# facebook/winterfell

Hardware: NVIDIA H100
Metric: prover_ms (lower is better)
Workload: dtype u64

## Files before the change

include/winterfell_b200.h:

```cpp
#ifndef WINTERFELL_B200_H
#define WINTERFELL_B200_H

#include <stddef.h>
#include <stdint.h>

#ifdef __cplusplus
extern "C" {
#endif

#define WF_OK 0
#define WF_ERR_CUDA (-1)
#define WF_ERR_INVALID (-2)
#define WF_ERR_UNSUPPORTED (-3)
#define WF_ERR_STATE (-4)

#define WF_HASH_BLAKE3_256 0
#define WF_HASH_RP64_256 1
#define WF_HASH_RPJIVE64_256 2
#define WF_HASH_SHA3_256 4
#define WF_HASH_BLAKE3_192 3

typedef struct wf_ctx wf_ctx;
typedef struct wf_mat wf_mat;
typedef struct wf_tree wf_tree;
// ... 62 lines not shown
typedef int (*wf_aux_builder_fn)(void* user, const uint64_t* rand_elements, uint64_t* aux_out);
int wf_prove_air_aux(wf_ctx* ctx, const uint64_t* air_desc, size_t air_desc_len, const uint64_t* const* trace_cols, int mont,
                     uint32_t log_n, const uint32_t* opts, wf_aux_builder_fn aux_builder, void* aux_user, uint8_t* proof,
                     size_t* proof_len);

typedef int (*wf_aux_assertions_fn)(void* user, const uint64_t* rand_elements, uint64_t* values);
int wf_prove_air_aux_dyn(wf_ctx* ctx, const uint64_t* air_desc, size_t air_desc_len, const uint64_t* const* trace_cols, int mont,
                         uint32_t log_n, const uint32_t* opts, wf_aux_builder_fn aux_builder, wf_aux_assertions_fn aux_assertions,
                         void* aux_user, uint8_t* proof, size_t* proof_len);

int wf_prove_fib_dev(wf_ctx* ctx, const uint64_t* d_trace, uint32_t k, uint32_t log_n, const uint64_t* results,
                     const uint32_t* opts, uint8_t* proof, size_t* proof_len);

int wf_aux_build_check(const uint64_t* air_desc, size_t air_desc_len, const uint64_t* aux_build, size_t aux_build_len, uint32_t log_n,
                       char* msg, size_t msg_cap);
int wf_aux_build(wf_ctx* ctx, const uint64_t* air_desc, size_t air_desc_len, const uint64_t* aux_build, size_t aux_build_len,
                 const wf_mat* main_evals, const uint64_t* rand, uint32_t ext, wf_mat** aux);
int wf_prove_air_aux_built(wf_ctx* ctx, const uint64_t* air_desc, size_t air_desc_len, const uint64_t* aux_build, size_t aux_build_len,
                           const uint64_t* const* trace_cols, const uint64_t* d_trace, int mont, uint32_t log_n, const uint32_t* opts,
                           wf_aux_assertions_fn aux_assertions, void* aux_user, uint8_t* proof, size_t* proof_len);

int wf_eval_constraints(wf_ctx* ctx, const uint64_t* air_desc, size_t air_desc_len, uint32_t log_n, uint32_t blowup, uint32_t ext,
                        const wf_mat* main_lde, const wf_mat* aux_lde, const uint64_t* coeffs, const uint64_t* aux_rand,
                        wf_mat** out);
int wf_composition_commit(wf_ctx* ctx, int hash_id, const wf_mat* comp_trace, uint32_t log_n, uint32_t blowup, uint32_t ext,
                          uint32_t num_cols, wf_mat** polys, wf_mat** lde, wf_tree** tree);
int wf_composition_commit_partitioned(wf_ctx* ctx, int hash_id, const wf_mat* comp_trace, uint32_t log_n, uint32_t blowup,
                                      uint32_t ext, uint32_t num_cols, uint32_t partition_size, wf_mat** polys, wf_mat** lde,
                                      wf_tree** tree);
int wf_mat_evaluate_at(wf_ctx* ctx, const wf_mat* polys, uint32_t ext, uint32_t col_ext, const uint64_t* z0, const uint64_t* z1,
                       uint64_t* out0, uint64_t* out1);
int wf_deep_compose(wf_ctx* ctx, uint32_t ext, const wf_mat* main_lde, const wf_mat* aux_lde, const wf_mat* cons_lde, uint32_t log_n,
                    const uint64_t* z, const uint64_t* coeffs, const uint64_t* ood_cur, const uint64_t* ood_next, wf_mat** out);

int wf_grind(wf_ctx* ctx, int hash_id, const uint8_t seed[32], uint32_t grinding, uint64_t* nonce);

typedef struct wf_comm {
    void* user;
    int rank, world;
    int (*exchange)(void* user, size_t nsend, const int* send_peer, const void* const* send, size_t nrecv,
                    const int* recv_peer, void* const* recv, size_t bytes);
    int (*all_gather_host)(void* user, const void* send, void* recv, size_t bytes);
    int (*all_reduce_sum)(void* user, void* d_buf, size_t words);
    int (*fork)(void* user);
    int (*join)(void* user);
} wf_comm;
int wf_prove_fib_sharded(wf_ctx* ctx, const wf_comm* comm, const uint64_t* const* local_cols, const uint64_t* d_local, int mont,
                         uint32_t k, uint32_t log_n, const uint64_t* results, const uint32_t* opts, uint8_t* proof,
                         size_t* proof_len, double* stats);

int wf_ctx_set_jit(wf_ctx* ctx, int on);
int wf_ctx_jit_stats(wf_ctx* ctx, uint64_t* compiled, uint64_t* cache_hits, uint64_t* fallbacks);
int wf_jit_compile_air(const uint64_t* air_desc, size_t air_desc_len, uint32_t ext, size_t* cubin_bytes, char* log, size_t log_cap);
int wf_air_check(const uint64_t* air_desc, size_t air_desc_len, uint32_t log_n, uint32_t blowup, char* msg, size_t msg_cap);

int wf_ntt_dev(wf_ctx* ctx, uint64_t* d_data, uint32_t log_n, uint32_t cols, int inverse);
int wf_hash_rows_dev(wf_ctx* ctx, int hash_id, const uint64_t* d_rows, size_t nrows, uint32_t cols, uint8_t* d_digests);
int wf_merkle_dev(wf_ctx* ctx, int hash_id, const uint8_t* d_leaves, size_t nleaves, uint8_t* d_nodes);
int wf_fri_fold_dev(wf_ctx* ctx, const uint64_t* d_evals, size_t len, int ext_degree, uint32_t folding_factor,
                    const uint64_t* alpha, uint64_t* d_next);

#define WF_FIELD_TEST_SHIFTS {1, 3, 6, 12, 24, 31, 32, 33, 48, 63, 64, 65, 72, 80, 84, 90, 95, 96}
int wf_field_ops_dev(wf_ctx* ctx, const uint64_t* d_a, const uint64_t* d_b, size_t n, uint64_t* d_out);
int wf_ext_ops_dev(wf_ctx* ctx, uint32_t ext, const uint64_t* d_a, const uint64_t* d_b, size_t n, uint64_t* d_out);

int wf_host_hash_elements(int hash_id, const uint64_t* elems, size_t n, uint8_t out[32]);
// ... 19 lines not shown
```

winterfell_b200/__init__.py:

```python
import ctypes as C
import os

import numpy as np

_HERE = os.path.dirname(os.path.abspath(__file__))
LIB_PATH = os.environ.get("WF_LIB_PATH") or os.path.join(_HERE, "libwinterfell_b200.so")

P = 0xFFFFFFFF00000001
HASH_BLAKE3_256 = 0
HASH_RP64_256 = 1
HASH_RPJIVE64_256 = 2
HASH_BLAKE3_192 = 3
HASH_SHA3_256 = 4

WF_OK = 0

u64p = C.POINTER(C.c_uint64)
u8p = C.POINTER(C.c_uint8)
vp = C.c_void_p

FRI_COMMIT_FN = C.CFUNCTYPE(None, C.c_void_p, u8p)
FRI_DRAW_FN = C.CFUNCTYPE(None, C.c_void_p, u64p)
AUX_BUILDER = C.CFUNCTYPE(C.c_int, C.c_void_p, u64p, u64p)

# ... 25 lines not shown
    ("wf_mat_wrap_device", C.c_int, [vp, vp, C.c_size_t, C.c_uint32, C.POINTER(vp)]),
    ("wf_trace_lde_from_host", C.c_int, [vp, C.POINTER(u64p), C.c_uint32, C.c_size_t, C.c_int, C.c_uint32, C.POINTER(vp), C.POINTER(vp)]),
    ("wf_mat_interpolate_with_offset", C.c_int, [vp, vp, C.c_uint64, C.POINTER(vp)]),
    ("wf_commit_rows", C.c_int, [vp, C.c_int, vp, C.POINTER(vp)]),
    ("wf_commit_rows_partitioned", C.c_int, [vp, C.c_int, vp, C.c_uint32, C.POINTER(vp)]),
    ("wf_tree_from_leaves", C.c_int, [vp, C.c_int, vp, C.c_size_t, C.c_int, C.POINTER(vp)]),
    ("wf_tree_free", C.c_int, [vp, vp]),
    ("wf_tree_root", C.c_int, [vp, vp, u8p]),
    ("wf_tree_num_leaves", C.c_size_t, [vp]),
    ("wf_tree_to_host", C.c_int, [vp, vp, u8p, u8p]),
    ("wf_tree_open_many", C.c_int, [vp, vp, u64p, C.c_size_t, u8p, u8p, C.POINTER(C.c_size_t)]),
    ("wf_fri_build_layers", C.c_int, [vp, C.c_int, vp, C.c_int, C.c_uint32, C.c_uint32, C.c_uint32, FRI_COMMIT_FN, FRI_DRAW_FN, vp, C.POINTER(vp)]),
    ("wf_fri_build_layers_default_channel", C.c_int, [vp, C.c_int, vp, C.c_int, C.c_uint32, C.c_uint32, C.c_uint32, u8p, C.c_size_t, C.POINTER(vp)]),
    ("wf_fri_num_layers", C.c_uint32, [vp]),
    ("wf_fri_remainder", C.c_size_t, [vp, u64p, C.c_size_t]),
    ("wf_fri_build_proof", C.c_int, [vp, vp, u64p, C.c_size_t, u8p, C.POINTER(C.c_size_t)]),
    ("wf_fri_free", C.c_int, [vp, vp]),
    ("wf_prove_fib", C.c_int, [vp, C.POINTER(u64p), C.c_int, C.c_uint32, C.c_uint32, u64p, C.POINTER(C.c_uint32), u8p, C.POINTER(C.c_size_t)]),
    ("wf_prove_air", C.c_int, [vp, u64p, C.c_size_t, C.POINTER(u64p), C.c_int, C.c_uint32, C.POINTER(C.c_uint32), u8p, C.POINTER(C.c_size_t)]),
    ("wf_prove_air_aux", C.c_int, [vp, u64p, C.c_size_t, C.POINTER(u64p), C.c_int, C.c_uint32, C.POINTER(C.c_uint32), AUX_BUILDER, vp,
                                   u8p, C.POINTER(C.c_size_t)]),
        ("wf_prove_air_aux_dyn", C.c_int, [vp, u64p, C.c_size_t, C.POINTER(u64p), C.c_int, C.c_uint32, C.POINTER(C.c_uint32), AUX_BUILDER, AUX_BUILDER, vp,
                                   u8p, C.POINTER(C.c_size_t)]),
    ("wf_aux_build_check", C.c_int, [u64p, C.c_size_t, u64p, C.c_size_t, C.c_uint32, C.c_char_p, C.c_size_t]),
    ("wf_aux_build", C.c_int, [vp, u64p, C.c_size_t, u64p, C.c_size_t, vp, u64p, C.c_uint32, C.POINTER(vp)]),
    ("wf_prove_air_aux_built", C.c_int, [vp, u64p, C.c_size_t, u64p, C.c_size_t, C.POINTER(u64p), vp, C.c_int, C.c_uint32,
                                         C.POINTER(C.c_uint32), AUX_BUILDER, vp, u8p, C.POINTER(C.c_size_t)]),
    ("wf_eval_constraints", C.c_int, [vp, u64p, C.c_size_t, C.c_uint32, C.c_uint32, C.c_uint32, vp, vp, u64p, u64p, C.POINTER(vp)]),
    ("wf_composition_commit", C.c_int, [vp, C.c_int, vp, C.c_uint32, C.c_uint32, C.c_uint32, C.c_uint32, C.POINTER(vp), C.POINTER(vp), C.POINTER(vp)]),
    ("wf_composition_commit_partitioned", C.c_int, [vp, C.c_int, vp, C.c_uint32, C.c_uint32, C.c_uint32, C.c_uint32, C.c_uint32, C.POINTER(vp),
                                                    C.POINTER(vp), C.POINTER(vp)]),
    ("wf_mat_evaluate_at", C.c_int, [vp, vp, C.c_uint32, C.c_uint32, u64p, u64p, u64p, u64p]),
    ("wf_deep_compose", C.c_int, [vp, C.c_uint32, vp, vp, vp, C.c_uint32, u64p, u64p, u64p, u64p, C.POINTER(vp)]),
    ("wf_prove_fib_dev", C.c_int, [vp, vp, C.c_uint32, C.c_uint32, u64p, C.POINTER(C.c_uint32), u8p, C.POINTER(C.c_size_t)]),
    ("wf_grind", C.c_int, [vp, C.c_int, u8p, C.c_uint32, C.POINTER(C.c_uint64)]),
    ("wf_ntt_dev", C.c_int, [vp, vp, C.c_uint32, C.c_uint32, C.c_int]),
    ("wf_hash_rows_dev", C.c_int, [vp, C.c_int, vp, C.c_size_t, C.c_uint32, vp]),
    ("wf_merkle_dev", C.c_int, [vp, C.c_int, vp, C.c_size_t, vp]),
    ("wf_fri_fold_dev", C.c_int, [vp, vp, C.c_size_t, C.c_int, C.c_uint32, u64p, vp]),
    ("wf_field_ops_dev", C.c_int, [vp, vp, vp, C.c_size_t, vp]),
    ("wf_ext_ops_dev", C.c_int, [vp, C.c_uint32, vp, vp, C.c_size_t, vp]),
    ("wf_ctx_set_jit", C.c_int, [vp, C.c_int]),
    ("wf_ctx_jit_stats", C.c_int, [vp, C.POINTER(C.c_uint64), C.POINTER(C.c_uint64), C.POINTER(C.c_uint64)]),
    ("wf_jit_compile_air", C.c_int, [u64p, C.c_size_t, C.c_uint32, C.POINTER(C.c_size_t), C.c_char_p, C.c_size_t]),
    ("wf_air_check", C.c_int, [u64p, C.c_size_t, C.c_uint32, C.c_uint32, C.c_char_p, C.c_size_t]),
    ("wf_host_hash_elements", C.c_int, [C.c_int, u64p, C.c_size_t, u8p]),
    ("wf_host_merge", C.c_int, [C.c_int, u8p, u8p]),
    ("wf_host_merge_with_int", C.c_int, [C.c_int, u8p, C.c_uint64, u8p]),
    ("wf_host_mul", C.c_uint64, [C.c_uint64, C.c_uint64]),
    ("wf_host_mul_2exp", C.c_uint64, [C.c_uint64, C.c_uint32]),
    ("wf_host_mont_to_canonical", C.c_uint64, [C.c_uint64]),
    ("wf_host_canonical_to_mont", C.c_uint64, [C.c_uint64]),
    ("wf_host_write_usize", C.c_size_t, [C.c_uint64, u8p]),
    ("wf_host_coin_draw", C.c_int, [C.c_int, u64p, C.c_size_t, u8p, C.c_int, C.c_size_t, u64p]),
    ("wf_host_build_fib_trace", C.c_int, [C.c_uint32, C.c_size_t, u64p, u64p]),
    ("wf_host_sharded_opening_plan", C.c_long, [C.c_size_t, C.c_int, C.c_int, u64p, C.c_size_t, u64p, u64p, C.c_size_t]),
    ("wf_prove_fib_sharded", C.c_int, [vp, vp, C.POINTER(u64p), vp, C.c_int, C.c_uint32, C.c_uint32, u64p, C.POINTER(C.c_uint32), u8p,
                                       C.POINTER(C.c_size_t), C.POINTER(C.c_double)]),
]


def declared_symbols():
    return [s[0] for s in _SIGS]


def lib():
# ... 117 lines not shown
        d_, dp = _u64(desc)
        c_, cp = _u64(coeffs)
        rp = None
        if aux_rand is not None:
            r_, rp = _u64(aux_rand)
        h = vp()
        self.check(self.L.wf_eval_constraints(self.h, dp, d_.size, log_n, blowup, ext, main_lde.h, aux_lde.h if aux_lde else None,
                                              cp, rp, C.byref(h)))
        return Mat(self, h)

    def composition_commit(self, hash_id, comp_trace, log_n, blowup, ext, num_cols):
        a, b, t = vp(), vp(), vp()
        self.check(self.L.wf_composition_commit(self.h, hash_id, comp_trace.h, log_n, blowup, ext, num_cols,
                                                C.byref(a), C.byref(b), C.byref(t)))
        return Mat(self, a), Mat(self, b), Tree(self, t)

    def evaluate_at(self, polys, ext, col_ext, z0, z1):
        a_, ap = _u64(z0)
        b_, bp = _u64(z1)
        ncols = polys.cols // col_ext
        o0 = np.zeros((ncols, ext), dtype=np.uint64)
        o1 = np.zeros((ncols, ext), dtype=np.uint64)
        self.check(self.L.wf_mat_evaluate_at(self.h, polys.h, ext, col_ext, ap, bp, o0.ctypes.data_as(u64p), o1.ctypes.data_as(u64p)))
        return o0, o1

    def deep_compose(self, ext, main_lde, aux_lde, cons_lde, log_n, z, coeffs, ood_cur, ood_next):
        z_, zp = _u64(z)
        c_, cp = _u64(coeffs)
        a_, ap = _u64(ood_cur)
        b_, bp = _u64(ood_next)
        h = vp()
        self.check(self.L.wf_deep_compose(self.h, ext, main_lde.h, aux_lde.h if aux_lde else None, cons_lde.h, log_n, zp, cp, ap, bp,
                                          C.byref(h)))
        return Mat(self, h)

    def prove_fib(self, trace, results, opts, mont=False, out_buf=None):
        a = np.ascontiguousarray(trace, dtype=np.uint64)
        c, n = a.shape
        ptrs = (u64p * c)(*[a[j].ctypes.data_as(u64p) for j in range(c)])
        r_, rp = _u64(results)
        o_ = np.ascontiguousarray(opts, dtype=np.uint32)
        buf = out_buf if out_buf is not None else np.zeros(1 << 23, dtype=np.uint8)
        cap = buf.size
        ln = C.c_size_t(cap)
        self.check(self.L.wf_prove_fib(self.h, ptrs, int(mont), c // 2, int(n).bit_length() - 1, rp,
                                       o_.ctypes.data_as(C.POINTER(C.c_uint32)), buf.ctypes.data_as(u8p), C.byref(ln)))
        return buf[: ln.value].tobytes()

    def prove_air(self, desc, trace, opts, mont=False):
        d_, dp = _u64(desc)
        a = np.ascontiguousarray(trace, dtype=np.uint64)
        c, n = a.shape
        ptrs = (u64p * c)(*[a[j].ctypes.data_as(u64p) for j in range(c)])
        o_ = np.ascontiguousarray(opts, dtype=np.uint32)
        cap = 1 << 23
        buf = np.zeros(cap, dtype=np.uint8)
        ln = C.c_size_t(cap)
        self.check(self.L.wf_prove_air(self.h, dp, d_.size, ptrs, int(mont), int(n).bit_length() - 1,
                                       o_.ctypes.data_as(C.POINTER(C.c_uint32)), buf.ctypes.data_as(u8p), C.byref(ln)))
        return buf[: ln.value].tobytes()

    def prove_air_aux(self, desc, trace, opts, builder, aux_width, num_rands, mont=False):
        d_, dp = _u64(desc)
        a = np.ascontiguousarray(trace, dtype=np.uint64)
        c, n = a.shape
        ptrs = (u64p * c)(*[a[j].ctypes.data_as(u64p) for j in range(c)])
# ... 343 lines not shown
```

winterfell_b200/csrc/prover.cu:

```cuda
#include <algorithm>
#include <chrono>

#include "internal.hpp"
#include "blake3.cuh"
#include "alg_hash.cuh"

#include "constraints_generic.cuh"

#ifndef FIB_ROWS_D3
#define FIB_ROWS_D3 2
#endif
struct FibEvalParams {
    SegMatrix lde;
    SegMatrix out;
    u32 k, log_n, log_blowup, log_ce_blowup;
    const u64* coef;
    u64 K0[3], K1[3];
    const u64* tw_ce;
    u64 zt[8];
    u64 last;
    size_t row0, ce_rows;
};

template <int D>
// ... 232 lines not shown
            for (int q = 0; q < 8; q++) {
                u32 j = g * 8 + q;
                if (j < p.c) {
#pragma unroll
                    for (int d = 0; d < D; d++) acc_mad(acc[d], s_t[(size_t)j * D + d], v[q]);
                }
            }
        }
    } else {
        for (u32 j = 0; j < p.c; j++) {
            const u64 v = seg_at(p.trace, row, j);
#pragma unroll
            for (int d = 0; d < D; d++) acc_mad(acc[d], s_t[(size_t)j * D + d], v);
        }
    }
    GlExt<D> S;
#pragma unroll
    for (int d = 0; d < D; d++) S.v[d] = acc_reduce(acc[d]);
    for (u32 j = 0; j < p.aw; j++) {
        GlExt<D> av;
#pragma unroll
        for (int q = 0; q < D; q++) av.v[q] = seg_at(p.aux, row, j * D + q);
        S = ext_add(S, ext_mul(ld_ext<D>(s_a + (size_t)j * D), av));
    }
    for (u32 j = 0; j < p.kc; j++) {
        GlExt<D> hv;
#pragma unroll
        for (int q = 0; q < D; q++) hv.v[q] = seg_at(p.cons, row, j * D + q);
        S = ext_add(S, ext_mul(ld_ext<D>(s_c + (size_t)j * D), hv));
    }
    u64* o = p.out.base + row * p.out.W;
#pragma unroll
    for (int q = 0; q < D; q++) o[q] = S.v[q];
}

#ifndef DEEP_ROWS1
#define DEEP_ROWS1 8
#endif
#ifndef DEEP_ROWS2
#define DEEP_ROWS2 8
#endif
#ifndef DEEP_ROWS3
#define DEEP_ROWS3 8
#endif
#ifndef DEEP_DIV_MINB
#define DEEP_DIV_MINB 2
#endif
#define DEEP_ROWS (D == 1 ? DEEP_ROWS1 : (D == 2 ? DEEP_ROWS2 : DEEP_ROWS3))
template <int D>
struct DeepPoint {
    u64 t, s, n;
    GlExt<D> q1, q0;
};
template <int D>
__device__ __forceinline__ u64 deep_m(const DeepPoint<D>& pt, u64 x, u64 x2) {
    if (D == 1) return gl_sub(x, pt.n);
    if (D == 2) return gl_add(gl_sub(x2, gl_mul(pt.t, x)), pt.n);
    return gl_sub(gl_add(gl_mul(x2, gl_sub(x, pt.t)), gl_mul(pt.s, x)), pt.n);
}
template <int D>
__device__ __forceinline__ GlExt<D> deep_q(const DeepPoint<D>& pt, u64 x, u64 x2) {
    GlExt<D> q;
    if (D == 1) { q.v[0] = 1; return q; }
    if (D == 2) { q = ext_sub(ext_from_base<D>(x), pt.q0); return q; }
    q = ext_sub(pt.q0, ext_mul_base(pt.q1, x));
    q.v[0] = gl_add(q.v[0], x2);
// ... 31 lines not shown
    for (int r = 0; r < ROWS; r++) {
        size_t row = tid + r * stride;
        if (row >= N) continue;
        u64* o = p.out.base + row * p.out.W;
        const GlExt<D> S = ld_ext<D>(o);
        const u64 x = D > 1 ? xs[r] : 0, x2 = D > 1 ? gl_sqr(x) : 0;
        const GlExt<D> a = ext_mul_base(ext_mul(ext_sub(S, Sz), deep_q<D>(pz, x, x2)), den[2 * r]);
        const GlExt<D> b = ext_mul_base(ext_mul(ext_sub(S, Szg), deep_q<D>(pzg, x, x2)), den[2 * r + 1]);
        const GlExt<D> v = ext_add(a, b);
#pragma unroll
        for (int q = 0; q < D; q++) o[q] = v.v[q];
    }
}
template <int D>
static bool deep_point(const GlExt<D>& z, DeepPoint<D>& pt) {
    pt.t = pt.s = pt.n = 0;
    pt.q1 = ext_zero<D>(); pt.q0 = ext_zero<D>();
    if (D == 1) { pt.n = z.v[0]; return true; }
    const GlExt<D> z1 = ext_frobenius(z);
    if (D == 2) {
        const GlExt<D> tr = ext_add(z, z1), nm = ext_mul(z, z1);
        pt.t = tr.v[0]; pt.n = nm.v[0]; pt.q0 = z1;
        return tr.v[1] == 0 && nm.v[1] == 0;
    }
    const GlExt<D> z2 = ext_frobenius(z1);
    const GlExt<D> tr = ext_add(z, ext_add(z1, z2));
    const GlExt<D> z12 = ext_mul(z1, z2);
    const GlExt<D> sm = ext_add(ext_mul(z, ext_add(z1, z2)), z12), nm = ext_mul(z, z12);
    pt.t = tr.v[0]; pt.s = sm.v[0]; pt.n = nm.v[0];
    pt.q1 = ext_add(z1, z2); pt.q0 = z12;
    bool ok = true;
    for (int k = 1; k < D; k++) ok = ok && tr.v[k] == 0 && sm.v[k] == 0 && nm.v[k] == 0;
    return ok;
}

__global__ void __launch_bounds__(256) grind_kernel(int hash_id, const u64* seed , u64 start, u64 count, u32 grinding,
                                                    unsigned long long* result) {
    u64 idx = (u64)blockIdx.x * blockDim.x + threadIdx.x;
    if (idx >= count) return;
    u64 nonce = start + idx;
    u64 head;
    if (WF_HASH_IS_BLAKE3(hash_id)) {
        u32 ws[8], cv[8];
#pragma unroll
        for (int i = 0; i < 4; i++) { ws[2 * i] = (u32)seed[i]; ws[2 * i + 1] = (u32)(seed[i] >> 32); }
        if (hash_id == WF_HASH_BLAKE3_256) b3_merge_with_int_words<8>(ws, nonce, cv, b3_runtime_one());
        else b3_merge_with_int_words<6>(ws, nonce, cv, b3_runtime_one());
        head = (u64)cv[0] | ((u64)cv[1] << 32);
    } else {
        u64 sd[4], o[4];
#pragma unroll
        for (int i = 0; i < 4; i++) sd[i] = seed[i];
        if (hash_id == WF_HASH_RP64_256) alg_merge_with_int<WF_HASH_RP64_256>(sd, nonce, o);
        else if (hash_id == WF_HASH_SHA3_256) alg_merge_with_int<WF_HASH_SHA3_256>(sd, nonce, o);
        else alg_merge_with_int<WF_HASH_RPJIVE64_256>(sd, nonce, o);
        head = o[0];
    }
    u64 mask = grinding >= 64 ? ~0ULL : ((1ULL << grinding) - 1);
    if ((head & mask) == 0) atomicMin(result, (unsigned long long)nonce);
}

static int grind_on_device(wf_ctx* ctx, int hash_id, const Digest& seed, u32 grinding, u64* nonce_out) {
    if (grinding == 0) { *nonce_out = 1; return WF_OK; }
    void *d_seed, *d_res;
    CKI(wf_dev_alloc(ctx, 32, &d_seed));
    CKI(wf_dev_alloc(ctx, 8, &d_res));
// ... 554 lines not shown
    CK(cudaGetLastError());
    wf_mat_free(ctx, ccoefs);
    wf_mark(ctx, "composition_interpolate");
    *polys_out = cpolys;
    return WF_OK;
}
int composition_commit(wf_ctx* ctx, int h, const wf_mat* comp, u32 log_n, u32 log_b, int D, u32 kc, wf_mat** polys_out,
                       wf_mat** lde_out, wf_tree** tree_out, u32 partition_words = 0) {
    wf_mat *cpolys = nullptr, *clde = nullptr;
    CKI(composition_polys(ctx, comp, log_n, D, kc, &cpolys));
    int r = wf_mat_lde(ctx, cpolys, log_b, &clde);
    if (r == WF_OK) {
        wf_mark(ctx, "composition_lde");
        if (tree_out) r = wf_commit_rows_partitioned(ctx, h, clde, partition_words, tree_out);
    }
    if (r != WF_OK) { wf_mat_free(ctx, cpolys); wf_mat_free(ctx, clde); return r; }
    *polys_out = cpolys;
    *lde_out = clde;
    return WF_OK;
}

template <int D>
int deep_compose(wf_ctx* ctx, const wf_mat* lde, const wf_mat* alde, const wf_mat* clde, u32 kc, u32 log_N,
                 const std::vector<GlExt<D>>& dc, const GlExt<D>& z, const GlExt<D>& zg, const GlExt<D>& Sz, const GlExt<D>& Szg,
                 wf_mat** out, size_t row0 = 0, size_t nrows = 0) {
    const u32 c = lde->m.cols, aw = alde ? alde->m.cols / D : 0, ct = c + aw;
    const size_t N = nrows ? nrows : ((size_t)1 << log_N);
    u64 *d_dt, *d_dq, *d_da;
    CKI(upload_ext<D>(ctx, dc, 0, ct + kc, &d_dt));
    d_da = d_dt + (size_t)c * D;
    d_dq = d_dt + (size_t)ct * D;
    wf_mat* deep;
    CKI(wf_mat_alloc(ctx, N, D, &deep));
    if (deep->m.W > D) CK(cudaMemsetAsync(deep->m.base, 0, deep->m.words() * 8, ctx->st));
    DeepParams p;
    p.trace = lde->m; p.cons = clde->m; p.out = deep->m; p.c = c; p.kc = kc; p.log_N = log_N;
    p.row0 = row0; p.nrows = nrows;
    p.tcc = d_dt; p.ccc = d_dq; p.acc = d_da; p.aw = aw;
    p.aux = aw ? alde->m : lde->m;
    CKI(wf_get_twiddles(ctx, log_N, &p.tw_N));
    const size_t coef_bytes = (size_t)(c + aw + kc) * D * 8;
    deep_sum_kernel<D><<<(unsigned)((N + DEEP_SUM_THREADS - 1) / DEEP_SUM_THREADS), DEEP_SUM_THREADS, coef_bytes, ctx->st>>>(p);
    const size_t rows_per_thread = DEEP_ROWS;
    size_t threads = (N + rows_per_thread - 1) / rows_per_thread;
    DeepPoint<D> pz, pzg;
    if (!deep_point<D>(z, pz) || !deep_point<D>(zg, pzg)) return wf_fail(ctx, WF_ERR_STATE, "conjugates of the out-of-domain point are inconsistent");
    deep_div_kernel<D><<<(unsigned)((threads + 255) / 256), 256, 0, ctx->st>>>(p, pz, pzg, Sz, Szg);
    ctx->launches += 2;
    CK(cudaGetLastError());
    wf_dev_free(ctx, d_dt);
    *out = deep;
    return WF_OK;
}

struct ProofScope {
    wf_ctx* ctx;
    std::vector<wf_mat**> mats;
    std::vector<wf_tree**> trees;
    wf_fri** fri = nullptr;
    explicit ProofScope(wf_ctx* c) : ctx(c) {}
    void own(std::initializer_list<wf_mat**> l) { mats.insert(mats.end(), l); }
    void own(std::initializer_list<wf_tree**> l) { trees.insert(trees.end(), l); }
    void drop(wf_mat*& m) { wf_mat_free(ctx, m); m = nullptr; }
    ~ProofScope() {
        if (fri && *fri) wf_fri_free(ctx, *fri);
        for (wf_mat** m : mats) if (*m) wf_mat_free(ctx, *m);
        for (wf_tree** t : trees) if (*t) wf_tree_free(ctx, *t);
    }
};

template <int D>
int prove_air(wf_ctx* ctx, const AirHost& air_in, const uint64_t* const* trace_cols, const uint64_t* d_trace, int mont, u32 log_n,
              const Options& o, wf_aux_builder_fn aux_builder, void* aux_user, std::vector<u8>& proof_out,
              wf_aux_assertions_fn aux_assertions = nullptr, const AuxBuildHost* aux_build = nullptr) {
    AirHost air_dyn;
    if (aux_assertions) air_dyn = air_in;
    const AirHost& air = aux_assertions ? air_dyn : air_in;
    const int h = o.hash_id;
    const size_t n = (size_t)1 << log_n;
    u32 log_b = 0;
    while ((1u << log_b) < o.blowup) log_b++;
    const size_t N = n << log_b;
    const u32 c = air.w, kc = air.num_comp_cols(n), log_ceb = air.log_ce_blowup();
    const u32 aw = air.aw, n_atr = (u32)air.aux_degrees.size(), n_aas = (u32)air.aux_asserts.size();
    const u32 n_mtr = (u32)air.degrees.size(), n_mas = (u32)air.asserts.size();
// ... 104 lines not shown
    }
    std::vector<GlExt<D>>&t_cur = ood[0], &t_nxt = ood[1], &qb_cur = ood[2], &qb_nxt = ood[3];
    auto combine = [&](const std::vector<GlExt<D>>& comp_evals) {
        std::vector<GlExt<D>> r(comp_evals.size() / D);
        for (u32 j = 0; j < r.size(); j++) {
            GlExt<D> acc = ext_zero<D>();
            for (int q = 0; q < D; q++) {
                GlExt<D> basis = ext_zero<D>();
                basis.v[q] = 1;
                acc = ext_add(acc, ext_mul(basis, comp_evals[j * D + q]));
            }
            r[j] = acc;
        }
        return r;
    };
    std::vector<GlExt<D>> q_cur = combine(qb_cur), q_nxt = combine(qb_nxt);
    if (aw) {
        auto a_cur = combine(ood[4]), a_nxt = combine(ood[5]);
        t_cur.insert(t_cur.end(), a_cur.begin(), a_cur.end());
        t_nxt.insert(t_nxt.end(), a_nxt.begin(), a_nxt.end());
    }
    const u32 ct = c + aw;
    ByteVec ood_t, ood_q;
    ood_t.u8_(2); write_elems<D>(ood_t, t_cur); write_elems<D>(ood_t, t_nxt);
    ood_q.u8_(2); write_elems<D>(ood_q, q_cur); write_elems<D>(ood_q, q_nxt);
    {
        ByteVec m;
        write_elems<D>(m, t_cur); write_elems<D>(m, q_cur); write_elems<D>(m, t_nxt); write_elems<D>(m, q_nxt);
        Digest dg = hh_hash_elements(h, (const u64*)m.v.data(), m.v.size() / 8);
        ch.coin.reseed(dg);
    }
    wf_mark(ctx, "ood_frames");
    std::vector<GlExt<D>> dc = ch.draw_coeffs(o.batch_d, ct + kc);
    GlExt<D> Sz = ext_zero<D>(), Szg = ext_zero<D>();
    for (u32 j = 0; j < ct; j++) { Sz = ext_add(Sz, ext_mul(dc[j], t_cur[j])); Szg = ext_add(Szg, ext_mul(dc[j], t_nxt[j])); }
    for (u32 j = 0; j < kc; j++) { Sz = ext_add(Sz, ext_mul(dc[ct + j], q_cur[j])); Szg = ext_add(Szg, ext_mul(dc[ct + j], q_nxt[j])); }
    CKI(deep_compose<D>(ctx, lde, alde, clde, kc, log_n + log_b, dc, z, zg, Sz, Szg, &deep));
    wf_mark(ctx, "deep_composition");
    {
        std::vector<Digest> fri_roots;
        CKI(wf_fri_build_layers_coin(ctx, h, deep, D, o.folding, o.rem_max_deg, o.blowup, ch.coin, fri_roots, &fri));
        for (auto& r : fri_roots) ch.commitments.bytes(r.b, WF_DIGEST_BYTES(h));
    }
    scope.drop(deep);
    wf_mark(ctx, "fri_layers");
    u64 nonce;
    CKI(grind_on_device(ctx, h, ch.coin.seed, o.grinding, &nonce));
    if (ch.coin.check_leading_zeros(nonce) < o.grinding) return wf_fail(ctx, WF_ERR_STATE, "grinding self-check failed");
    std::vector<u64> pos;
    if (!ch.coin.draw_integers(o.num_queries, N, nonce, pos)) return wf_fail(ctx, WF_ERR_STATE, "failed to draw query positions");
    std::sort(pos.begin(), pos.end());
    pos.erase(std::unique(pos.begin(), pos.end()), pos.end());
    wf_mark(ctx, "grinding");
    ByteVec w;
    w.u8_((u8)c); w.u8_((u8)aw); w.u8_((u8)air.nr); w.u8_((u8)log_n); w.u16_(0);
    w.u8_(8); w.u64_(GL_P);
    w.u8_((u8)o.num_queries); w.u8_((u8)o.blowup); w.u8_((u8)o.grinding); w.u8_((u8)o.ext); w.u8_((u8)o.folding);
    w.u8_((u8)o.rem_max_deg); w.u8_((u8)o.batch_c); w.u8_((u8)o.batch_d); w.u8_((u8)o.num_partitions); w.u8_((u8)o.hash_rate);
    w.usize(n_tr + n_as);
    w.u8_((u8)pos.size());
    w.u16_((uint16_t)ch.commitments.v.size());
    w.bytes(ch.commitments.v.data(), ch.commitments.v.size());
    GatherBatch gb;
    FriProofPlan fplan;
    size_t tr_rows = gb.add_rows(lde->m, pos), cr_rows = gb.add_rows(clde->m, pos), tr_dig, cr_dig;
    size_t ar_rows = 0, ar_dig = 0;
    if (aw) ar_rows = gb.add_rows(alde->m, pos);
    CKI(gb.add_opening(ctx, ttree, pos, &tr_dig));
    CKI(gb.add_opening(ctx, ctree, pos, &cr_dig));
    if (aw) CKI(gb.add_opening(ctx, atree, pos, &ar_dig));
// ... 796 lines not shown

template <int D>
static int deep_entry(wf_ctx* ctx, const wf_mat* lde, const wf_mat* alde, const wf_mat* clde, u32 log_n, const uint64_t* zw,
                      const uint64_t* coeffs, const uint64_t* ood_cur, const uint64_t* ood_next, wf_mat** out) {
    const u32 c = lde->m.cols, aw = alde ? alde->m.cols / D : 0, kc = clde->m.cols / D, tot = c + aw + kc;
    u32 log_N = 0;
    while (((size_t)1 << log_N) < lde->m.rows) log_N++;
    if (log_n > log_N) return wf_fail(ctx, WF_ERR_INVALID, "trace length exceeds the LDE domain");
    std::vector<GlExt<D>> dc(tot);
    GlExt<D> z = ext_zero<D>(), Sz = ext_zero<D>(), Szg = ext_zero<D>();
    for (int q = 0; q < D; q++) z.v[q] = zw[q];
    for (u32 i = 0; i < tot; i++) {
        GlExt<D> a = ext_zero<D>(), b = ext_zero<D>();
        for (int q = 0; q < D; q++) { dc[i].v[q] = coeffs[i * D + q]; a.v[q] = ood_cur[i * D + q]; b.v[q] = ood_next[i * D + q]; }
        Sz = ext_add(Sz, ext_mul(dc[i], a));
        Szg = ext_add(Szg, ext_mul(dc[i], b));
    }
    GlExt<D> zg = ext_mul_base(z, gl_root_of_unity(log_n));
    return deep_compose<D>(ctx, lde, alde, clde, kc, log_N, dc, z, zg, Sz, Szg, out);
}
extern "C" int wf_deep_compose(wf_ctx* ctx, uint32_t ext, const wf_mat* main_lde, const wf_mat* aux_lde, const wf_mat* cons_lde,
                               uint32_t log_n, const uint64_t* z, const uint64_t* coeffs, const uint64_t* ood_cur,
                               const uint64_t* ood_next, wf_mat** out) {
    if (!ctx || !main_lde || !cons_lde || !z || !coeffs || !ood_cur || !ood_next || !out || ext < 1 || ext > 3 ||
        cons_lde->m.cols % ext || cons_lde->m.rows != main_lde->m.rows || (aux_lde && (aux_lde->m.cols % ext || aux_lde->m.rows != main_lde->m.rows)))
        return wf_fail(ctx, WF_ERR_INVALID, "bad arguments");
    switch (ext) {
        case 1: return deep_entry<1>(ctx, main_lde, aux_lde, cons_lde, log_n, z, coeffs, ood_cur, ood_next, out);
        case 2: return deep_entry<2>(ctx, main_lde, aux_lde, cons_lde, log_n, z, coeffs, ood_cur, ood_next, out);
        default: return deep_entry<3>(ctx, main_lde, aux_lde, cons_lde, log_n, z, coeffs, ood_cur, ood_next, out);
    }
}

extern "C" int wf_prove_fib_sharded(wf_ctx* ctx, const wf_comm* comm, const uint64_t* const* local_cols, const uint64_t* d_local, int mont,
                                    uint32_t k, uint32_t log_n, const uint64_t* results, const uint32_t* opts, uint8_t* proof,
                                    size_t* proof_len, double* stats) {
    if (!ctx || !comm || !comm->exchange || !comm->all_gather_host || !comm->all_reduce_sum || (!local_cols && !d_local) || !results ||
        !opts || !proof || !proof_len || k == 0 || 2 * k > 255 || log_n < 3)
        return wf_fail(ctx, WF_ERR_INVALID, "bad arguments");
    Options o;
    CKI(parse_options(ctx, opts, o));
    std::vector<u8> out;
    int r;
    switch (o.ext) {
        case 1: r = prove_fib_sharded<1>(ctx, comm, local_cols, d_local, mont, k, log_n, results, o, out, stats); break;
        case 2: r = prove_fib_sharded<2>(ctx, comm, local_cols, d_local, mont, k, log_n, results, o, out, stats); break;
        default: r = prove_fib_sharded<3>(ctx, comm, local_cols, d_local, mont, k, log_n, results, o, out, stats); break;
    }
    if (r != WF_OK) return r;
    if (out.size() > *proof_len) return wf_fail(ctx, WF_ERR_INVALID, "proof buffer too small (%zu needed)", out.size());
    memcpy(proof, out.data(), out.size());
    *proof_len = out.size();
    return WF_OK;
}
extern "C" int wf_prove_fib(wf_ctx* ctx, const uint64_t* const* trace_cols, int mont, uint32_t k, uint32_t log_n,
                            const uint64_t* results, const uint32_t* opts, uint8_t* proof, size_t* proof_len) {
    return prove_fib_entry(ctx, trace_cols, nullptr, mont, k, log_n, results, opts, proof, proof_len);
}
extern "C" int wf_prove_fib_dev(wf_ctx* ctx, const uint64_t* d_trace, uint32_t k, uint32_t log_n, const uint64_t* results,
                                const uint32_t* opts, uint8_t* proof, size_t* proof_len) {
    return prove_fib_entry(ctx, nullptr, d_trace, 0, k, log_n, results, opts, proof, proof_len);
}
```

Before: 92.41.

## Compute DEEP composition in coefficient form via synthetic division, then LDE

Instead of evaluating the DEEP composition pointwise over the full LDE domain, it linearly combines the trace and constraint polynomial coefficients at size n. It then divides by (x-z) and (x-zg) using a parallel synthetic-division scan (reduce, carry, apply kernels), and runs one LDE of the resulting quotient. This moves the heavy per-row work from blowup·n rows to n rows, trading it for an extra NTT and three scan kernels. The explicit zeroing memset of the output padding is replaced by in-kernel zeroing.

Result: faster. 87.70 (median of 6 runs) (-5.1%).

```diff
diff --git a/include/winterfell_b200.h b/include/winterfell_b200.h
--- a/include/winterfell_b200.h
+++ b/include/winterfell_b200.h
@@ -118,6 +118,8 @@
                        uint64_t* out0, uint64_t* out1);
 int wf_deep_compose(wf_ctx* ctx, uint32_t ext, const wf_mat* main_lde, const wf_mat* aux_lde, const wf_mat* cons_lde, uint32_t log_n,
                     const uint64_t* z, const uint64_t* coeffs, const uint64_t* ood_cur, const uint64_t* ood_next, wf_mat** out);
+int wf_deep_compose_polys(wf_ctx* ctx, uint32_t ext, const wf_mat* main_polys, const wf_mat* aux_polys, const wf_mat* cons_polys,
+                          uint32_t log_blowup, const uint64_t* z, const uint64_t* coeffs, wf_mat** out);
 
 int wf_grind(wf_ctx* ctx, int hash_id, const uint8_t seed[32], uint32_t grinding, uint64_t* nonce);
 
diff --git a/winterfell_b200/__init__.py b/winterfell_b200/__init__.py
--- a/winterfell_b200/__init__.py
+++ b/winterfell_b200/__init__.py
@@ -81,6 +81,7 @@
                                                     C.POINTER(vp), C.POINTER(vp)]),
     ("wf_mat_evaluate_at", C.c_int, [vp, vp, C.c_uint32, C.c_uint32, u64p, u64p, u64p, u64p]),
     ("wf_deep_compose", C.c_int, [vp, C.c_uint32, vp, vp, vp, C.c_uint32, u64p, u64p, u64p, u64p, C.POINTER(vp)]),
+    ("wf_deep_compose_polys", C.c_int, [vp, C.c_uint32, vp, vp, vp, C.c_uint32, u64p, u64p, C.POINTER(vp)]),
     ("wf_prove_fib_dev", C.c_int, [vp, vp, C.c_uint32, C.c_uint32, u64p, C.POINTER(C.c_uint32), u8p, C.POINTER(C.c_size_t)]),
     ("wf_grind", C.c_int, [vp, C.c_int, u8p, C.c_uint32, C.POINTER(C.c_uint64)]),
     ("wf_ntt_dev", C.c_int, [vp, vp, C.c_uint32, C.c_uint32, C.c_int]),
@@ -264,6 +265,14 @@
         h = vp()
         self.check(self.L.wf_deep_compose(self.h, ext, main_lde.h, aux_lde.h if aux_lde else None, cons_lde.h, log_n, zp, cp, ap, bp,
                                           C.byref(h)))
+        return Mat(self, h)
+
+    def deep_compose_polys(self, ext, main_polys, aux_polys, cons_polys, log_blowup, z, coeffs):
+        z_, zp = _u64(z)
+        c_, cp = _u64(coeffs)
+        h = vp()
+        self.check(self.L.wf_deep_compose_polys(self.h, ext, main_polys.h, aux_polys.h if aux_polys else None, cons_polys.h,
+                                                log_blowup, zp, cp, C.byref(h)))
         return Mat(self, h)
 
     def prove_fib(self, trace, results, opts, mont=False, out_buf=None):
diff --git a/winterfell_b200/csrc/prover.cu b/winterfell_b200/csrc/prover.cu
--- a/winterfell_b200/csrc/prover.cu
+++ b/winterfell_b200/csrc/prover.cu
@@ -288,6 +288,7 @@
     u64* o = p.out.base + row * p.out.W;
 #pragma unroll
     for (int q = 0; q < D; q++) o[q] = S.v[q];
+    for (int q = D; q < p.out.W; q++) o[q] = 0;
 }
 
 #ifndef DEEP_ROWS1
@@ -385,6 +386,171 @@
     bool ok = true;
     for (int k = 1; k < D; k++) ok = ok && tr.v[k] == 0 && sm.v[k] == 0 && nm.v[k] == 0;
     return ok;
+}
+
+#define SYN_THREADS 256
+#define SYN_ITEMS 8
+#define SYN_TILE (SYN_THREADS * SYN_ITEMS)
+template <int D>
+struct SynDivParams {
+    GlExt<D> b[2];
+    GlExt<D> b_items[2];
+    GlExt<D> b_tile[2];
+};
+template <int D>
+struct SynRun {
+    GlExt<D> a[2], p[2];
+};
+template <int D>
+__device__ __forceinline__ SynRun<D> syn_ident() {
+    SynRun<D> r;
+#pragma unroll
+    for (int pt = 0; pt < 2; pt++) { r.a[pt] = ext_zero<D>(); r.p[pt] = ext_from_base<D>(1); }
+    return r;
+}
+template <int D>
+__device__ __forceinline__ SynRun<D> syn_cat(const SynRun<D>& lo, const SynRun<D>& hi) {
+    SynRun<D> r;
+#pragma unroll
+    for (int pt = 0; pt < 2; pt++) { r.a[pt] = ext_add(lo.a[pt], ext_mul(lo.p[pt], hi.a[pt])); r.p[pt] = ext_mul(lo.p[pt], hi.p[pt]); }
+    return r;
+}
+template <int D>
+__device__ __forceinline__ SynRun<D> syn_shfl_down(const SynRun<D>& v, u32 off) {
+    SynRun<D> r;
+#pragma unroll
+    for (int pt = 0; pt < 2; pt++)
+#pragma unroll
+        for (int q = 0; q < D; q++) {
+            r.a[pt].v[q] = __shfl_down_sync(0xffffffffu, v.a[pt].v[q], off);
+            r.p[pt].v[q] = __shfl_down_sync(0xffffffffu, v.p[pt].v[q], off);
+        }
+    return r;
+}
+template <int D>
+__device__ __forceinline__ SynRun<D> syn_block_suffix(const SynRun<D>& v, SynRun<D>& total) {
+    constexpr u32 NW = SYN_THREADS / 32;
+    __shared__ SynRun<D> wrun[NW];
+    const u32 lane = threadIdx.x & 31, wid = threadIdx.x >> 5;
+    SynRun<D> x = v;
+#pragma unroll
+    for (u32 off = 1; off < 32; off <<= 1) {
+        const SynRun<D> y = syn_shfl_down(x, off);
+        if (lane + off < 32) x = syn_cat(x, y);
+    }
+    if (lane == 0) wrun[wid] = x;
+    __syncthreads();
+    if (wid == 0) {
+        SynRun<D> s = lane < NW ? wrun[lane] : syn_ident<D>();
+#pragma unroll
+        for (u32 off = 1; off < NW; off <<= 1) {
+            const SynRun<D> y = syn_shfl_down(s, off);
+            if (lane + off < NW) s = syn_cat(s, y);
+        }
+        if (lane < NW) wrun[lane] = s;
+    }
+    __syncthreads();
+    total = wrun[0];
+    SynRun<D> ex = syn_shfl_down(x, 1);
+    if (lane == 31) ex = syn_ident<D>();
+    if (wid + 1 < NW) ex = syn_cat(ex, wrun[wid + 1]);
+    __syncthreads();
+    return ex;
+}
+template <int D>
+__device__ __forceinline__ GlExt<D> syn_ld(const u64* m, size_t i) {
+    GlExt<D> r;
+    if constexpr (D == 1) {
+        r.v[0] = m[i];
+    } else {
+        const ulonglong2 lo = *reinterpret_cast<const ulonglong2*>(m + i * (D == 3 ? 4 : 2));
+        r.v[0] = lo.x; r.v[1] = lo.y;
+        if constexpr (D == 3) r.v[2] = m[i * 4 + 2];
+    }
+    return r;
+}
+template <int D>
+__device__ __forceinline__ void syn_st(u64* m, size_t i, const GlExt<D>& v) {
+    if constexpr (D == 1) {
+        m[i] = v.v[0];
+    } else if constexpr (D == 2) {
+        *reinterpret_cast<ulonglong2*>(m + i * 2) = make_ulonglong2(v.v[0], v.v[1]);
+    } else {
+        ulonglong2* o = reinterpret_cast<ulonglong2*>(m + i * 4);
+        o[0] = make_ulonglong2(v.v[0], v.v[1]);
+        o[1] = make_ulonglong2(v.v[2], 0);
+    }
+}
+template <int D>
+__device__ __forceinline__ SynRun<D> syn_thread_run(const u64* m, size_t n, size_t r0, const SynDivParams<D>& sp) {
+    SynRun<D> r;
+#pragma unroll
+    for (int pt = 0; pt < 2; pt++) { r.a[pt] = ext_zero<D>(); r.p[pt] = sp.b_items[pt]; }
+#pragma unroll
+    for (int k = SYN_ITEMS - 1; k >= 0; k--) {
+        const GlExt<D> s = r0 + k < n ? syn_ld<D>(m, r0 + k) : ext_zero<D>();
+#pragma unroll
+        for (int pt = 0; pt < 2; pt++) r.a[pt] = ext_add(s, ext_mul(sp.b[pt], r.a[pt]));
+    }
+    return r;
+}
+template <int D>
+__global__ void __launch_bounds__(SYN_THREADS) syn_div_reduce(const u64* s, size_t n, SynDivParams<D> sp, u64* agg ) {
+    const size_t r0 = (size_t)blockIdx.x * SYN_TILE + (size_t)threadIdx.x * SYN_ITEMS;
+    SynRun<D> total;
+    syn_block_suffix<D>(syn_thread_run<D>(s, n, r0, sp), total);
+    if (threadIdx.x == 0) {
+#pragma unroll
+        for (int pt = 0; pt < 2; pt++)
+#pragma unroll
+            for (int q = 0; q < D; q++) agg[((size_t)blockIdx.x * 2 + pt) * D + q] = total.a[pt].v[q];
+    }
+}
+template <int D>
+__global__ void __launch_bounds__(SYN_THREADS) syn_div_carry(u64* agg, size_t ntiles, SynDivParams<D> sp) {
+    const size_t per = (ntiles + SYN_THREADS - 1) / SYN_THREADS;
+    const size_t b = threadIdx.x * per < ntiles ? threadIdx.x * per : ntiles, e = b + per < ntiles ? b + per : ntiles;
+    SynRun<D> mine;
+#pragma unroll
+    for (int pt = 0; pt < 2; pt++) { mine.a[pt] = ext_zero<D>(); mine.p[pt] = ext_from_base<D>(1); }
+    for (size_t i = e; i-- > b;) {
+#pragma unroll
+        for (int pt = 0; pt < 2; pt++) {
+            mine.a[pt] = ext_add(ld_ext<D>(agg + (i * 2 + pt) * D), ext_mul(sp.b_tile[pt], mine.a[pt]));
+            mine.p[pt] = ext_mul(sp.b_tile[pt], mine.p[pt]);
+        }
+    }
+    SynRun<D> total;
+    const SynRun<D> above = syn_block_suffix<D>(mine, total);
+    GlExt<D> run[2] = {above.a[0], above.a[1]};
+    for (size_t i = e; i-- > b;) {
+#pragma unroll
+        for (int pt = 0; pt < 2; pt++) {
+            u64* g = agg + (i * 2 + pt) * D;
+            const GlExt<D> a = ld_ext<D>(g);
+#pragma unroll
+            for (int q = 0; q < D; q++) g[q] = run[pt].v[q];
+            run[pt] = ext_add(a, ext_mul(sp.b_tile[pt], run[pt]));
+        }
+    }
+}
+template <int D>
+__global__ void __launch_bounds__(SYN_THREADS) syn_div_apply(u64* s, size_t n, SynDivParams<D> sp, const u64* carry) {
+    const size_t r0 = (size_t)blockIdx.x * SYN_TILE + (size_t)threadIdx.x * SYN_ITEMS;
+    SynRun<D> total;
+    const SynRun<D> above = syn_block_suffix<D>(syn_thread_run<D>(s, n, r0, sp), total);
+    GlExt<D> q[2];
+#pragma unroll
+    for (int pt = 0; pt < 2; pt++) q[pt] = ext_add(above.a[pt], ext_mul(above.p[pt], ld_ext<D>(carry + ((size_t)blockIdx.x * 2 + pt) * D)));
+#pragma unroll
+    for (int k = SYN_ITEMS - 1; k >= 0; k--) {
+        const size_t i = r0 + k;
+        if (i >= n) continue;
+        const GlExt<D> si = syn_ld<D>(s, i);
+        syn_st<D>(s, i, ext_add(q[0], q[1]));
+#pragma unroll
+        for (int pt = 0; pt < 2; pt++) q[pt] = ext_add(si, ext_mul(sp.b[pt], q[pt]));
+    }
 }
 
 __global__ void __launch_bounds__(256) grind_kernel(int hash_id, const u64* seed , u64 start, u64 count, u32 grinding,
@@ -1005,7 +1171,6 @@
     d_dq = d_dt + (size_t)ct * D;
     wf_mat* deep;
     CKI(wf_mat_alloc(ctx, N, D, &deep));
-    if (deep->m.W > D) CK(cudaMemsetAsync(deep->m.base, 0, deep->m.words() * 8, ctx->st));
     DeepParams p;
     p.trace = lde->m; p.cons = clde->m; p.out = deep->m; p.c = c; p.kc = kc; p.log_N = log_N;
     p.row0 = row0; p.nrows = nrows;
@@ -1024,6 +1189,39 @@
     wf_dev_free(ctx, d_dt);
     *out = deep;
     return WF_OK;
+}
+
+template <int D>
+int deep_compose_polys(wf_ctx* ctx, const wf_mat* polys, const wf_mat* apolys, const wf_mat* cpolys, u32 kc, u32 log_b,
+                       const std::vector<GlExt<D>>& dc, const GlExt<D>& z, const GlExt<D>& zg, wf_mat** out) {
+    const u32 c = polys->m.cols, aw = apolys ? apolys->m.cols / D : 0, ct = c + aw;
+    const size_t n = polys->m.rows, ntiles = (n + SYN_TILE - 1) / SYN_TILE;
+    u32 log_n = 0;
+    while (((size_t)1 << log_n) < n) log_n++;
+    DevScratch tmp(ctx);
+    u64* d_dt;
+    CKI(upload_ext<D>(ctx, dc, 0, ct + kc, &d_dt));
+    tmp.bufs.push_back(d_dt);
+    void* d_agg;
+    CKI(tmp.alloc(ntiles * 2 * D * 8, &d_agg));
+    wf_mat* quot;
+    CKI(wf_mat_alloc(ctx, n, D, &quot));
+    DeepParams p{};
+    p.trace = polys->m; p.cons = cpolys->m; p.out = quot->m; p.c = c; p.kc = kc; p.log_N = log_n;
+    p.tcc = d_dt; p.acc = d_dt + (size_t)c * D; p.ccc = d_dt + (size_t)ct * D; p.aw = aw;
+    p.aux = aw ? apolys->m : polys->m;
+    deep_sum_kernel<D><<<(unsigned)((n + DEEP_SUM_THREADS - 1) / DEEP_SUM_THREADS), DEEP_SUM_THREADS, (size_t)(ct + kc) * D * 8, ctx->st>>>(p);
+    SynDivParams<D> sp;
+    sp.b[0] = z; sp.b[1] = zg;
+    for (int pt = 0; pt < 2; pt++) { sp.b_items[pt] = ext_pow(sp.b[pt], SYN_ITEMS); sp.b_tile[pt] = ext_pow(sp.b[pt], SYN_TILE); }
+    syn_div_reduce<D><<<(unsigned)ntiles, SYN_THREADS, 0, ctx->st>>>(quot->m.base, n, sp, (u64*)d_agg);
+    syn_div_carry<D><<<1, SYN_THREADS, 0, ctx->st>>>((u64*)d_agg, ntiles, sp);
+    syn_div_apply<D><<<(unsigned)ntiles, SYN_THREADS, 0, ctx->st>>>(quot->m.base, n, sp, (const u64*)d_agg);
+    ctx->launches += 4;
+    const cudaError_t e = cudaGetLastError();
+    const int r = e == cudaSuccess ? wf_mat_lde(ctx, quot, log_b, out) : wf_fail(ctx, WF_ERR_CUDA, "DEEP quotient launch: %s", cudaGetErrorString(e));
+    wf_mat_free(ctx, quot);
+    return r;
 }
 
 struct ProofScope {
@@ -1194,10 +1392,7 @@
     }
     wf_mark(ctx, "ood_frames");
     std::vector<GlExt<D>> dc = ch.draw_coeffs(o.batch_d, ct + kc);
-    GlExt<D> Sz = ext_zero<D>(), Szg = ext_zero<D>();
-    for (u32 j = 0; j < ct; j++) { Sz = ext_add(Sz, ext_mul(dc[j], t_cur[j])); Szg = ext_add(Szg, ext_mul(dc[j], t_nxt[j])); }
-    for (u32 j = 0; j < kc; j++) { Sz = ext_add(Sz, ext_mul(dc[ct + j], q_cur[j])); Szg = ext_add(Szg, ext_mul(dc[ct + j], q_nxt[j])); }
-    CKI(deep_compose<D>(ctx, lde, alde, clde, kc, log_n + log_b, dc, z, zg, Sz, Szg, &deep));
+    CKI(deep_compose_polys<D>(ctx, polys, apolys, cpolys, kc, log_b, dc, z, zg, &deep));
     wf_mark(ctx, "deep_composition");
     {
         std::vector<Digest> fri_roots;
@@ -2060,6 +2255,33 @@
     }
 }
 
+template <int D>
+static int deep_polys_entry(wf_ctx* ctx, const wf_mat* polys, const wf_mat* apolys, const wf_mat* cpolys, u32 log_n, u32 log_b,
+                            const uint64_t* zw, const uint64_t* coeffs, wf_mat** out) {
+    const u32 kc = cpolys->m.cols / D, tot = polys->m.cols + (apolys ? apolys->m.cols / D : 0) + kc;
+    std::vector<GlExt<D>> dc(tot);
+    GlExt<D> z = ext_zero<D>();
+    for (int q = 0; q < D; q++) z.v[q] = zw[q];
+    for (u32 i = 0; i < tot; i++) for (int q = 0; q < D; q++) dc[i].v[q] = coeffs[i * D + q];
+    return deep_compose_polys<D>(ctx, polys, apolys, cpolys, kc, log_b, dc, z, ext_mul_base(z, gl_root_of_unity(log_n)), out);
+}
+extern "C" int wf_deep_compose_polys(wf_ctx* ctx, uint32_t ext, const wf_mat* main_polys, const wf_mat* aux_polys, const wf_mat* cons_polys,
+                                     uint32_t log_blowup, const uint64_t* z, const uint64_t* coeffs, wf_mat** out) {
+    if (!ctx || !main_polys || !cons_polys || !z || !coeffs || !out || ext < 1 || ext > 3 || cons_polys->m.cols % ext ||
+        cons_polys->m.rows != main_polys->m.rows || (aux_polys && (aux_polys->m.cols % ext || aux_polys->m.rows != main_polys->m.rows)))
+        return wf_fail(ctx, WF_ERR_INVALID, "bad arguments");
+    const size_t n = main_polys->m.rows;
+    u32 log_n = 0;
+    while (((size_t)1 << log_n) < n) log_n++;
+    if (n < 8 || (n & (n - 1))) return wf_fail(ctx, WF_ERR_INVALID, "rows must be a power of two >= 8");
+    if (log_blowup < 1 || log_blowup > 7 || log_n + log_blowup > 32) return wf_fail(ctx, WF_ERR_INVALID, "bad blowup");
+    switch (ext) {
+        case 1: return deep_polys_entry<1>(ctx, main_polys, aux_polys, cons_polys, log_n, log_blowup, z, coeffs, out);
+        case 2: return deep_polys_entry<2>(ctx, main_polys, aux_polys, cons_polys, log_n, log_blowup, z, coeffs, out);
+        default: return deep_polys_entry<3>(ctx, main_polys, aux_polys, cons_polys, log_n, log_blowup, z, coeffs, out);
+    }
+}
+
 extern "C" int wf_prove_fib_sharded(wf_ctx* ctx, const wf_comm* comm, const uint64_t* const* local_cols, const uint64_t* d_local, int mont,
                                     uint32_t k, uint32_t log_n, const uint64_t* results, const uint32_t* opts, uint8_t* proof,
                                     size_t* proof_len, double* stats) {
```
